# daultanigaurav/AI-BASED-FRAME-INTERPOLATION

Hardware: AMD Instinct MI355X
Metric: interpolated frames/sec at 1080p (higher is better)
Workload: dtype bf16

## Files before the change

### ai_based_frame_interpolation_amd/_native.py

```python
from __future__ import annotations

import ctypes
import os
import subprocess

import torch

_PKG = os.path.dirname(os.path.abspath(__file__))
LIB_PATH = os.environ.get("FIUNET_LIB") or os.path.join(_PKG, "libfiunet_hip.so")
CSRC = os.path.join(_PKG, "csrc")

ABI_VERSION = 8
ABI_MIN_COMPAT = 4
FP32, BF16, BF16X2, FP16 = 0, 1, 2, 3
OPT_UNFUSED, OPT_KEEP_ALL, OPT_GATHER_UPSAMPLE = 1, 2, 16
OPT_RNE_WEIGHTS, OPT_NO_DITHER = 32, 64
YUV_MPEG2, YUV_BT709, YUV_FULL_RANGE, YUV_BT2020 = 1, 2, 4, 8

SYMBOLS = (
    "fiunet_abi_version", "fiunet_last_error_string", "fiunet_create", "fiunet_destroy",
    "fiunet_set_options", "fiunet_load_weights", "fiunet_prepare_precision", "fiunet_workspace_bytes", "fiunet_forward",
    "fiunet_min_unsplit_batch",
    "fiunet_forward_strip",
    "fiunet_workspace_bytes_u8", "fiunet_forward_u8", "fiunet_forward_u8_strided", "fiunet_preprocess_u8",
    "fiunet_postprocess_u8", "fiunet_debug_read_activation", "fiunet_profile_enable",
    "fiunet_profile_read", "fiunet_metrics_workspace_bytes", "fiunet_psnr_u8", "fiunet_ssim_u8",
    "fiunet_ssim_gauss_workspace_bytes", "fiunet_ssim_gauss_f32",
    "fiunet_yuv420_to_rgb_u8", "fiunet_rgb_to_yuv420_u8", "fiunet_workspace_bytes_yuv420", "fiunet_forward_yuv420",
    "fiunet_preprocess_p10", "fiunet_postprocess_p10", "fiunet_workspace_bytes_p10", "fiunet_forward_p10",
    "fiunet_yuv420p10_to_rgb_p10", "fiunet_rgb_p10_to_yuv420p10", "fiunet_workspace_bytes_yuv420p10",
    "fiunet_forward_yuv420p10",
    "fiunet_pair_sad_u8", "fiunet_pair_sad_p10", "fiunet_scene_cuts", "fiunet_hold_cut_frames",
    "fiunet_retime_u8", "fiunet_retime_p10",
    "fiunet_nv12_to_rgb_u8", "fiunet_rgb_to_nv12_u8", "fiunet_workspace_bytes_nv12", "fiunet_forward_nv12",
    "fiunet_p010_to_rgb_p10", "fiunet_rgb_p10_to_p010", "fiunet_workspace_bytes_p010", "fiunet_forward_p010",
)


class SurfaceLayout(ctypes.Structure):
# ... 421 lines not shown
```

### ai_based_frame_interpolation_amd/csrc/conv3x3_mfma.hip.h

```cpp
#pragma once
#include <hip/hip_runtime.h>
#include <stdint.h>
#include <type_traits>

namespace fiunet {

typedef __attribute__((ext_vector_type(4))) float f32x4;
typedef __attribute__((ext_vector_type(8))) __bf16 bf16x8;
typedef __attribute__((ext_vector_type(8))) _Float16 f16x8;

enum SrcMode { SRC_DIRECT = 0, SRC_POOL = 1 , SRC_CONCAT_UP = 2,
               SRC_STEM = 3 ,
               SRC_DIRECT_X2 = 4,
               SRC_STEM_X2 = 5 };
constexpr bool src_is_stem(int mode) { return mode == SRC_STEM || mode == SRC_STEM_X2; }
constexpr bool src_is_x2(int mode) { return mode == SRC_DIRECT_X2 || mode == SRC_STEM_X2; }

__device__ __forceinline__ size_t blk_off(int plane, int y, int x, int H, int W)
{
    return (((size_t)plane * H + y) * W + x) * 64;
}

struct ConvArgs {
    const void* src0;
// ... 9 lines not shown
    int padT, padL;
    float sy, sx;
    int upOffY;
    int lowOffY;
    int lowHg;
    int tilesX, tilesY, nct;
    int relu;
    const float* f1;
    const float* f2;
    const void* stem_w;
    float dither;
    int ksplit;
    float* kslab;
    unsigned long long* stamp;
    unsigned stamp_cap;
    const float* head_w;
    const float* head_b;
    float* head_out;
    const uint8_t* u1;
    const uint8_t* u2;
    uint8_t* head_out_u8;
    int head_nc;
    size_t head_img_stride;
};

template <typename T> struct Elem;
template <> struct Elem<float> {
    static constexpr int PL = 16;
    static constexpr int NE = 4;
};
template <> struct Elem<__bf16> {
    static constexpr int PL = 32;
    static constexpr int NE = 8;
};
template <> struct Elem<_Float16> {
    static constexpr int PL = 32;
    static constexpr int NE = 8;
};

template <typename T> __device__ __forceinline__ void chunk_unpack(const uint4& c, float* f);
template <> __device__ __forceinline__ void chunk_unpack<float>(const uint4& c, float* f)
{
    f[0] = __uint_as_float(c.x); f[1] = __uint_as_float(c.y);
    f[2] = __uint_as_float(c.z); f[3] = __uint_as_float(c.w);
}
template <> __device__ __forceinline__ void chunk_unpack<__bf16>(const uint4& c, float* f)
// ... 320 lines not shown
    static constexpr int TAB_BYTES = MODE == SRC_CONCAT_UP ? ((THP + TW + 2) * 16 + 255) / 256 * 256 : 0;
    static constexpr int STEMW_OFF = TAB_OFF + TAB_BYTES;
    static constexpr int STEMW_BYTES = src_is_stem(MODE) ? 4096 : 0;
    static constexpr int LDS_BYTES = STEMW_OFF + STEMW_BYTES;
    static_assert(LDS_BYTES <= 80 * 1024, "two workgroups must fit in the CU's 160 KiB of LDS");
    static_assert(!src_is_stem(MODE) || LDS_BYTES <= 63 * 1280, "fused-stem kernel: stay below 64 LDS granules");
};

constexpr int conv_wave_frags(int BN, int TH, int TW) { return TH * TW / 16 / (4 / (BN / 64)); }
constexpr int conv_occupancy(int BN, int TH, int TW, int lds_bytes = 0)
{
    return conv_wave_frags(BN, TH, TW) == 4 && lds_bytes * 3 <= 160 * 1024 ? 3 : 2;
}


__device__ __forceinline__ int conv_block_remap()
{
    const int nblk = gridDim.x, bid = blockIdx.x;
    const int q = nblk >> 3, r = nblk & 7, xcd = bid & 7;
    return (xcd < r ? xcd * (q + 1) : r * (q + 1) + (xcd - r) * q) + (bid >> 3);
}

struct ConvTileId { int ct, b, ty, tx; };
__device__ __forceinline__ ConvTileId conv_tile_decode(const ConvArgs& a, int t)
{
    ConvTileId d;
    d.ct = t % a.nct; t /= a.nct;
    d.tx = t % a.tilesX; t /= a.tilesX;
    d.ty = t % a.tilesY;
    d.b = t / a.tilesY;
    return d;
}

template <typename T> __device__ __forceinline__ int conv_cout_ofs(int m, int lc)
{
    return sizeof(T) == 2 ? (m >> 1) * 32 + lc * 8 + (m & 1) * 4 : m * 16 + lc * 4;
}

template <typename T, int BN, int TH, int TW, int EPI>
__device__ __forceinline__ void conv_acc_init(const ConvArgs& a, f32x4 (&acc)[4][conv_wave_frags(BN, TH, TW)],
                                              int ct, int wc, int lc)
{
    constexpr int NF = conv_wave_frags(BN, TH, TW);
#pragma unroll
    for (int m = 0; m < 4; ++m) {
        f32x4 v = f32x4{0.f, 0.f, 0.f, 0.f};
        if constexpr (!epi_is_splitk(EPI)) {
            const float4 sh = *reinterpret_cast<const float4*>(a.shift + ct * BN + wc * 64 + conv_cout_ofs<T>(m, lc));
            v = f32x4{sh.x, sh.y, sh.z, sh.w};
        }
#pragma unroll
        for (int n = 0; n < NF; ++n) acc[m][n] = v;
    }
}
// ... 263 lines not shown
            } else {
#pragma unroll
                for (int g = 0; g < 2; ++g) {
                    unsigned r[4];
#pragma unroll
                    for (int h = 0; h < 2; ++h) {
                        const int m = 2 * g + h;
                        const unsigned a0 = pk_max_i16(pack2_pk<T>(acc[m][n][0], acc[m][n][1]),
                                                       pack2_pk<T>(acc[m][n + FR][0], acc[m][n + FR][1]));
                        const unsigned a1 = pk_max_i16(pack2_pk<T>(acc[m][n][2], acc[m][n][3]),
                                                       pack2_pk<T>(acc[m][n + FR][2], acc[m][n + FR][3]));
                        r[2 * h] = pk_max_i16(a0, dpp_swap_pairs(a0));
                        r[2 * h + 1] = pk_max_i16(a1, dpp_swap_pairs(a1));
                        if (a.relu) { r[2 * h] = relu_pk_bf16(r[2 * h]); r[2 * h + 1] = relu_pk_bf16(r[2 * h + 1]); }
                    }
                    if (okp) *reinterpret_cast<uint4*>(o + g * pplane_stride) = make_uint4(r[0], r[1], r[2], r[3]);
                }
            }
        }
    }
}

template <typename T, int BN, int TH, int TW, int MODE, int EPI>
__global__ __launch_bounds__(256, conv_occupancy(BN, TH, TW, ConvTile<BN, TH, TW, MODE>::LDS_BYTES)) void conv3x3_mfma_kernel(const ConvArgs a)
{
    using Tile = ConvTile<BN, TH, TW, MODE>;
    constexpr int PL = Elem<T>::PL;
    constexpr int TWP = Tile::TWP, THP = Tile::THP;
    constexpr int WAVES_C = BN / 64, WAVES_P = 4 / WAVES_C;
    constexpr int FR = TW / 16;
    constexpr int NF = conv_wave_frags(BN, TH, TW);
    constexpr int ROWS_W = NF / FR;
    static_assert(NF == 8 || NF == 4, "wave tile must be 64 couts x 128 or 64 pixels");
    static_assert(TH == ROWS_W * WAVES_P && ROWS_W * FR == NF, "tile does not split over the waves");
    static_assert(EPI != EPI_POOL || ROWS_W % 2 == 0, "pooled epilogue: a wave owns whole row pairs");
    static_assert(Tile::LDS_BYTES * conv_occupancy(BN, TH, TW, Tile::LDS_BYTES) <= 160 * 1024, "LDS per CU");
    constexpr int HNC = EPI == EPI_HEAD ? 1 : (EPI == EPI_HEAD3 ? 3 : 0);
    static_assert(HNC == 0 || BN == 64, "fused head needs all 64 couts in one wave");
    static_assert(MODE == SRC_DIRECT || MODE == SRC_CONCAT_UP || MODE == SRC_STEM || MODE == SRC_DIRECT_X2 ||
                  MODE == SRC_STEM_X2, "pooling is fused into the producer");
    constexpr bool X2 = src_is_x2(MODE);
    constexpr bool STEM = src_is_stem(MODE);
    constexpr bool DIRECT = MODE == SRC_DIRECT || MODE == SRC_DIRECT_X2;
    static_assert(!X2 || std::is_same_v<T, __bf16>, "two-piece operands are bf16");
    static_assert(!STEM || (sizeof(T) == 2 && BN == 64), "fused stem: 2-byte output (bf16 / fp16), 64 couts");

    extern __shared__ __attribute__((aligned(16))) char smem[];
    char* const lds_in = smem;
    char* const lds_w = smem + Tile::IN_BYTES;
    const unsigned lds_in_addr = lds_addr_of(lds_in);
    const unsigned lds_w_addr = lds_addr_of(lds_w);

    int lid = conv_block_remap();
    const int ksplit = epi_is_splitk(EPI) ? a.ksplit : 1;
    const int split = lid % ksplit;
    lid /= ksplit;
    const ConvTileId id = conv_tile_decode(a, lid);
    const int ct = id.ct, b = id.b;
    const int y0 = id.ty * TH, x0 = id.tx * TW;

    const int tid = threadIdx.x;
    const int lane = tid & 63, wave = __builtin_amdgcn_readfirstlane(tid >> 6);
    const int l15 = lane & 15, lc = lane >> 4;
    const int wc = wave % WAVES_C, wp = wave / WAVES_C;

#ifdef FIUNET_STAMP
    unsigned long long st_sum[16] = {0, 0, 0, 0, 0, 0, 0, 0, 0, 0, 0, 0, 0, 0, 0, 0};
    unsigned long long st_t0 = __builtin_amdgcn_s_memtime(), st_prev = st_t0;
#ifdef FIUNET_STAMP_PROLOG
    unsigned long long st_pprev = st_t0;
#define PSTAMP(slot) do { __builtin_amdgcn_sched_barrier(0); const unsigned long long t_ = __builtin_amdgcn_s_memtime(); \
                          st_sum[slot] += t_ - st_pprev; st_pprev = t_; __builtin_amdgcn_sched_barrier(0); } while (0)
#else
#define PSTAMP(slot) do {} while (0)
#endif
#define STAMP(slot) do { const unsigned long long t_ = __builtin_amdgcn_s_memtime(); \
                         st_sum[slot] += t_ - st_prev; st_prev = t_; } while (0)
#define STAMP_UP(slot) STAMP(slot)
#else
#define STAMP(slot) do {} while (0)
#define STAMP_UP(slot) do {} while (0)
#define PSTAMP(slot) do {} while (0)
// ... 525 lines not shown
        const unsigned long long ck_t1 = __builtin_amdgcn_s_memtime(), ck_r1 = __builtin_amdgcn_s_memrealtime();
        const unsigned st_idx = blockIdx.x * 4u + (unsigned)wave;
        if (a.stamp && lane == 0 && st_idx < a.stamp_cap) {
            unsigned long long* rec = a.stamp + (size_t)st_idx * 16;
            rec[0] = ck_t1 - ck_t0;
            rec[1] = ck_r1 - ck_r0;
            rec[8] = 1ull;
        }
    }
#endif
    conv_epilogue<T, BN, TH, TW, EPI, X2>(a, acc, b, y0, x0, ct, split, wc, wp, l15, lc);
#ifdef FIUNET_STAMP
    STAMP(5);
    st_sum[0] = st_prev - st_t0;
    const unsigned st_idx = blockIdx.x * 4u + (unsigned)wave;
    if (a.stamp && lane == 0 && st_idx < a.stamp_cap) {
        unsigned long long* rec = a.stamp + (size_t)st_idx * 16;
#pragma unroll
        for (int k = 0; k < 16; ++k) rec[k] = k == 8 ? 1ull : st_sum[k];
    }
#endif
}

template <typename T, int BN, int TH, int TW, int EPI, bool X2>
__global__ __launch_bounds__(64) void splitk_finalize_tile_kernel(const ConvArgs a)
{
    static_assert(EPI == EPI_PLAIN || EPI == EPI_POOL, "a fused head is never K-split");
    constexpr int WAVES_C = BN / 64;
    constexpr int NF = conv_wave_frags(BN, TH, TW);
    int t = blockIdx.x >> 2;
    const int tile = t;
    const int ct = t % a.nct; t /= a.nct;
    const int tx = t % a.tilesX; t /= a.tilesX;
    const int ty = t % a.tilesY;
    const int b = t / a.tilesY;
    const int lane = threadIdx.x & 63, wave = blockIdx.x & 3;
    const int l15 = lane & 15, lc = lane >> 4;
    const int wc = wave % WAVES_C, wp = wave / WAVES_C;
    const int ntile = a.B * a.tilesY * a.tilesX * a.nct;
    f32x4 acc[4][NF];
#pragma unroll
    for (int m = 0; m < 4; ++m)
#pragma unroll
        for (int n = 0; n < NF; ++n) acc[m][n] = f32x4{0.f, 0.f, 0.f, 0.f};
    const float4* p = reinterpret_cast<const float4*>(a.kslab) + (((size_t)tile * 4 + wave) * (4 * NF)) * 64 + lane;
    const size_t slice = (size_t)ntile * 4 * (4 * NF) * 64;
// ... 36 lines not shown
```

### ai_based_frame_interpolation_amd/csrc/fiunet.hip

```cpp
#include "../../include/fiunet.h"
#include "pointwise.hip.h"
#include "conv3x3_kwave.hip.h"
#include "metrics.hip.h"
#include "colour.hip.h"
#include "scene.hip.h"
#include "retime.hip.h"

#include <algorithm>
#include <atomic>
#include <cmath>
#include <cstdio>
#include <cstring>
#include <map>
#include <string>
#include <vector>

using namespace fiunet;

namespace {

thread_local std::string g_err;

int fail(int code, const std::string& msg)
{
// ... 146 lines not shown
    if (dev >= 0 && dev < 64 && !lds_attr_set[dev].load(std::memory_order_acquire)) {
        HIP_TRY(hipFuncSetAttribute(reinterpret_cast<const void*>(Kernel), hipFuncAttributeMaxDynamicSharedMemorySize, lds));
        lds_attr_set[dev].store(true, std::memory_order_release);
    }
    hipLaunchKernelGGL(Kernel, dim3((unsigned)nblk), dim3(256), lds, s, a);
    HIP_TRY(hipGetLastError());
    return FIUNET_OK;
}

template <typename T, int BN, int TH, int TW, int MODE, int EPI>
int launch_conv_cfg(ConvArgs a, hipStream_t s)
{
    char name[128] = "";
    if (g_name_out)
        std::snprintf(name, sizeof name, "conv3x3_mfma_kernel<%s,%d,%d,%d,%d,%d>", elem_name<T>(), BN, TH, TW,
                      MODE, EPI);
    a.tilesX = (a.W + TW - 1) / TW;
    a.tilesY = (a.H + TH - 1) / TH;
    a.nct = a.Cout / BN;
    const long long nblk = (long long)a.B * a.tilesX * a.tilesY * a.nct * (epi_is_splitk(EPI) ? a.ksplit : 1);
    return launch_lds<&conv3x3_mfma_kernel<T, BN, TH, TW, MODE, EPI>>(name, nblk, ConvTile<BN, TH, TW, MODE>::LDS_BYTES, a, s);
}

inline unsigned grid_for(size_t n) { return (unsigned)std::min<size_t>((n + 255) / 256, 256 * 32); }

inline long long padded_area(int H, int W, int TH, int TW)
{
    return (long long)((H + TH - 1) / TH) * TH * ((W + TW - 1) / TW) * TW;
}

inline bool prefer_wide(int H, int W, int THw, int TWw, int THn, int TWn)
{
    const long long wide = padded_area(H, W, THw, TWw), narrow = padded_area(H, W, THn, TWn);
    return wide * 32 <= narrow * 33;
}

struct TileShape { int BN, TH, TW; };
struct ConvCfg { bool small; int ksplit; bool kwave = false; };

inline TileShape big_tile(int H, int W, int Cout)
{
    if (Cout == 64) return prefer_wide(H, W, 16, 32, 32, 16) ? TileShape{64, 16, 32} : TileShape{64, 32, 16};
    return prefer_wide(H, W, 8, 32, 16, 16) ? TileShape{128, 8, 32} : TileShape{128, 16, 16};
}
constexpr TileShape kSmallTile = {64, 8, 32};

inline long long tile_blocks(const TileShape& t, int B, int H, int W, int Cout)
{
    return (long long)B * ((W + t.TW - 1) / t.TW) * ((H + t.TH - 1) / t.TH) * (Cout / t.BN);
}

inline int pow2_floor(long long v) { int k = 1; while (2LL * k <= v) k *= 2; return k; }

inline int small_ksplit(bool fp32, long long nblk, int nplanes, int fp32_slots = 256)
{
    int k;
    if (nblk >= (fp32 ? fp32_slots : 256)) return 1;
    if (fp32) k = pow2_floor(std::max<long long>(1, fp32_slots / std::max<long long>(nblk, 1)));
    else {
        k = nplanes < 8 ? 1 : (nplanes < 16 ? 4 : 8);
        k = std::min(k, pow2_floor(std::max<long long>(1, 512 / std::max<long long>(nblk, 1))));
    }
    k = std::min(k, pow2_floor(nplanes));
    while (k > 1 && (size_t)k * nblk * kSmallTile.BN * kSmallTile.TH * kSmallTile.TW * 4 > kSlabBytes) k /= 2;
    return k;
}

inline bool kwave_applies(int B, int H, int W, int Cin, int Cout)
{
    const TileShape big = big_tile(H, W, Cout);
    const long long nblk_big = tile_blocks(big, B, H, W, Cout);
    if (nblk_big >= 256 || !(nblk_big < (nblk_big / B < 64 ? 256 : 128))) return false;
    const long long nwg = (long long)B * ((H + 1) / 2) * ((W + 31) / 32) * (Cout / 64);
    return Cin / 32 >= 4 && Cout % 64 == 0 && nwg <= 256;
}

inline bool small_tile_wins_on_the_tail(long long nblk_big, long long nblk_small, double area_ratio)
{
    auto rounds = [](long long n, int slots, int occ) {
        const long long full = n / slots, rem = n % slots;
        return (double)full + (rem ? 0.2 + 0.8 * (double)((rem + 255) / 256) / occ : 0.0);
    };
    return rounds(nblk_small, 768, 3) * 0.81 * area_ratio < rounds(nblk_big, 512, 2);
}

inline ConvCfg choose_conv_cfg(bool fp32, bool x2, int B, int H, int W, int Cin, int Cout, bool splittable,
                               int force_small = -1, int force_ksplit = 0, bool kwave_ok = false, bool tail_rule_ok = false,
                               bool concat_conv = false)
{
    const int PL = fp32 ? 16 : 32;
    const int nplanes = Cin / PL * (x2 ? 3 : 1);
    const TileShape big = big_tile(H, W, Cout);
    const long long nblk_big = tile_blocks(big, B, H, W, Cout), nblk_small = tile_blocks(kSmallTile, B, H, W, Cout);
    if (nblk_big >= 256 && force_small < 0 && force_ksplit <= 0) {
        const bool small = tail_rule_ok && nblk_big <= 2304 &&
                           small_tile_wins_on_the_tail(nblk_big, nblk_small,
                                                       (double)padded_area(H, W, kSmallTile.TH, kSmallTile.TW) /
                                                           (double)padded_area(H, W, big.TH, big.TW));
        return ConvCfg{small, 1};
    }
    const bool may_split = splittable && nblk_big < (nblk_big / B < 64 ? 256 : 128);
    if (kwave_ok && fp32 && splittable && Cin / 16 >= 4 && force_small == 2) return ConvCfg{true, 1, true};
    if (kwave_ok && !fp32 && splittable && Cin / 32 >= 4 && (force_small == 2 || (force_small < 0 && force_ksplit <= 0))) {
        if (force_small == 2 || (kwave_applies(B, H, W, Cin, Cout) && !(x2 && Cin / 32 > 8))) return ConvCfg{true, 1, true};
    }
    if (force_small == 2) force_small = 1;
    auto big_ksplit = [&]() {
        int k = (int)std::min<long long>(std::min(nplanes / 2, 16), (256 + nblk_big - 1) / nblk_big);
        k = k > 1 ? pow2_floor(k) : 1;
        while (k > 1 && (size_t)k * nblk_big * big.BN * big.TH * big.TW * 4 > kSlabBytes) k /= 2;
        return k;
    };
    bool small = force_small >= 0 ? force_small != 0 : true;
    if (force_small < 0 && fp32) {
        const int slots = concat_conv ? 512 : 256;
        auto mfma_ns = [&](long long nblk, int k, double step_ns) {
            const long long nwg = nblk * k;
            return (double)((nwg + slots - 1) / slots) * ((nplanes + k - 1) / k * 3) * step_ns + (k > 1 ? 8000.0 : 0.0);
        };
        const int ks = may_split ? small_ksplit(true, nblk_small, nplanes, slots) : 1, kb = may_split ? big_ksplit() : 1;
        small = mfma_ns(nblk_small, ks, 2950.0) <= mfma_ns(nblk_big, kb, 5900.0);
        if (kwave_ok && splittable && may_split && nplanes >= 4 && Cout % 64 == 0) {
            const long long nwg = (long long)B * ((H + 1) / 2) * ((W + 31) / 32) * (Cout / 64);
            const double kw = (double)((nwg + 255) / 256) * ((nplanes + 3) / 4 * 3) * 2950.0;
            if (nwg <= 512 && kw < (small ? mfma_ns(nblk_small, ks, 2950.0) : mfma_ns(nblk_big, kb, 5900.0))) return ConvCfg{true, 1, true};
        }
    }
    const TileShape& t = small ? kSmallTile : big;
    const long long nblk = small ? nblk_small : nblk_big;
    int k = 1;
    if (force_ksplit > 0) {
        k = splittable ? std::min(pow2_floor(force_ksplit), pow2_floor(nplanes)) : 1;
        while (k > 1 && (size_t)k * nblk * t.BN * t.TH * t.TW * 4 > kSlabBytes) k /= 2;
    } else if (may_split) {
        k = small ? small_ksplit(fp32, nblk, nplanes, concat_conv ? 512 : 256) : big_ksplit();
    }
    return ConvCfg{small, k};
}

inline bool fp32_concat_takes_kwave(int B, int H, int W, int Cin, int Cout)
{
    return choose_conv_cfg(true, false, B, H, W, Cin, Cout, true, -1, 0, true, false, false).kwave;
}

enum StemForm {
    STEM_FUSED = 0,
    STEM_FIRST = 1,
    STEM_RGB_SPLIT = 2,
};
enum SrcForm {
    FORM_DIRECT = 0,
    FORM_POOL = 1,
    FORM_CONCAT_GATHER = 2,
    FORM_CONCAT_UP = 3,
    FORM_CONCAT_CONVT = 4,
    FORM_CONCAT_UPCAT = 5,
    FORM_STEM = 6,
};
struct StageLaunch {
    int form = FORM_DIRECT;
// ... 11 lines not shown
    bool stem_w = false;
    const int* force_tile = nullptr;
    const int* force_ksplit = nullptr;
};

inline int conv_cin(const int* cout, bool bilinear, int i)
{
    if (kMode[i] != SRC_CONCAT_UP) return cout[kSrc0[i]];
    return cout[kSrc0[i]] + (bilinear ? cout[kSrc1[i]] : cout[kSrc1[i]] / 2);
}

inline bool materialise_up(int precision, int B, int H, int W, int Cin, int Cout)
{
    if (precision == FIUNET_FP32) return fp32_concat_takes_kwave(B, H, W, Cin, Cout);
    if (Cout >= 256 && (long long)B * H * W >= 65536) return true;
    return kwave_applies(B, H, W, Cin, Cout);
}

void plan_stages(const NetDesc& n, int precision, int B, int H, int W, StageLaunch L[NCONV])
{
    const bool fp32 = precision == FIUNET_FP32, x2 = precision == FIUNET_BF16X2;
    const bool keep_all = n.flags & FIUNET_OPT_KEEP_ALL;
    const bool unfused = !x2 && (n.flags & FIUNET_OPT_UNFUSED), gather_up = !x2 && (n.flags & FIUNET_OPT_GATHER_UPSAMPLE);
    int hs[5] = {H}, ws[5] = {W};
    for (int k = 1; k < 5; ++k) { hs[k] = hs[k - 1] / 2; ws[k] = ws[k - 1] / 2; }
    const bool fuse_stem = !fp32 && n.cf == 1 && n.stem_w && !unfused && !(x2 && keep_all) && prefer_wide(H, W, 16, 32, 32, 16);
    L[0] = StageLaunch{};
    L[0].form = fuse_stem && !keep_all ? STEM_FUSED : n.cf == 3 && !fp32 ? STEM_RGB_SPLIT : STEM_FIRST;
    L[0].stored = L[0].form != STEM_FUSED;
    for (int i = 1; i < NCONV; ++i) {
        StageLaunch& st = L[i];
        st = StageLaunch{};
        const int h = hs[kLevel[i]], w = ws[kLevel[i]], cin = conv_cin(n.cout, n.bilinear, i), cout = n.cout[i];
        if (i == 1 && fuse_stem) st.form = FORM_STEM;
        else if (kMode[i] == SRC_POOL) st.form = FORM_POOL;
        else if (kMode[i] == SRC_CONCAT_UP) {
            if (!n.bilinear) st.form = FORM_CONCAT_CONVT;
            else if (x2) st.form = FORM_CONCAT_UP;
            else if (unfused) st.form = FORM_CONCAT_UPCAT;
            else st.form = !gather_up && materialise_up(precision, B, h, w, cin, cout) ? FORM_CONCAT_UP : FORM_CONCAT_GATHER;
        }
        if (kPoolOut[i] >= 0 && !unfused) st.epi = EPI_POOL;
        if (i == NCONV - 1 && !unfused) st.epi = n.cf == 1 ? EPI_HEAD : EPI_HEAD3;
        st.slab = i != NCONV - 1;
        st.stored = !(i == NCONV - 1 && st.epi != EPI_PLAIN && !keep_all);
        const bool stem = st.form == FORM_STEM, gather = st.form == FORM_CONCAT_GATHER, direct = !stem && !gather;
        const bool plain_or_pool = st.epi == EPI_PLAIN || st.epi == EPI_POOL;
        const bool as_gather = st.form == FORM_CONCAT_UPCAT && fp32 && !fp32_concat_takes_kwave(B, h, w, cin, cout);
        st.cfg = choose_conv_cfg(fp32, x2, B, h, w, cin, cout, !stem && plain_or_pool && st.slab,
                                 (n.force_tile ? n.force_tile[i] : 0) - 1, stem || !n.force_ksplit ? 0 : n.force_ksplit[i],
                                 direct && plain_or_pool && !as_gather, direct || (gather && cout >= 256), gather || as_gather);
    }
}

struct Plan {
    StageLaunch st[NCONV];
    int hs[5], ws[5];
    size_t act_off[NCONV];
    size_t pool_off[4];
    size_t scratch_off;
    size_t up_off[NCONV];
    size_t slab_off;
    size_t total;
};

bool make_plan(const NetDesc& n, int B, int H, int W, int precision, Plan& p)
{
    if (B < 1 || H < 16 || W < 16) return false;
    if ((long long)H * W >= (1LL << 26)) return false;
    plan_stages(n, precision, B, H, W, p.st);
    const bool keep_all = n.flags & FIUNET_OPT_KEEP_ALL;
    const size_t es = two_byte_elems(precision) ? 2 : 4;
    p.hs[0] = H; p.ws[0] = W;
    for (int k = 1; k < 5; ++k) { p.hs[k] = p.hs[k - 1] / 2; p.ws[k] = p.ws[k - 1] / 2; }
// ... 70 lines not shown
            k.ksplit = ksplit;
            int rc = launch_conv_cfg<T, BN, TH, TW, MODE, EPI_SPLITK>(k, s);
            if (rc) return rc;
            k.tilesX = (a.W + TW - 1) / TW;
            k.tilesY = (a.H + TH - 1) / TH;
            k.nct = a.Cout / BN;
            const long long ntile = (long long)a.B * k.tilesX * k.tilesY * k.nct;
            hipLaunchKernelGGL((splitk_finalize_tile_kernel<T, BN, TH, TW, EPI, src_is_x2(MODE)>), dim3((unsigned)(4 * ntile)), dim3(64), 0, s, k);
            HIP_TRY(hipGetLastError());
            if (g_name_out) *g_name_out += "+splitk" + std::to_string(ksplit);
            return FIUNET_OK;
        }
    }
    return launch_conv_cfg<T, BN, TH, TW, MODE, EPI>(a, s);
}

template <typename T, int MODE, int EPI> int launch_conv_shape(const ConvArgs& a, const ConvCfg& cfg, hipStream_t s)
{
    if (a.Cout != 64 && a.Cout % 128 != 0) return fail(FIUNET_ERR_INVALID_ARG, "Cout must be 64 or k*128");
    if ((EPI == EPI_HEAD || EPI == EPI_HEAD3) && a.Cout != 64) return fail(FIUNET_ERR_INVALID_ARG, "fused head needs Cout == 64");
    if constexpr ((MODE == SRC_DIRECT || MODE == SRC_DIRECT_X2) && (EPI == EPI_PLAIN || EPI == EPI_POOL)) {
        if (cfg.kwave) return launch_kwave<T, EPI, MODE == SRC_DIRECT_X2>(a, s);
    }
    if (cfg.small) return launch_conv_maybe_split<T, 64, 8, 32, MODE, EPI>(a, s, cfg.ksplit);
    if (a.Cout == 64) {
        const bool wide = prefer_wide(a.H, a.W, 16, 32, 32, 16);
        return wide ? launch_conv_maybe_split<T, 64, 16, 32, MODE, EPI>(a, s, cfg.ksplit)
                    : launch_conv_maybe_split<T, 64, 32, 16, MODE, EPI>(a, s, cfg.ksplit);
    }
    if constexpr (EPI != EPI_HEAD && EPI != EPI_HEAD3) {
        const bool wide = prefer_wide(a.H, a.W, 8, 32, 16, 16);
        return wide ? launch_conv_maybe_split<T, 128, 8, 32, MODE, EPI>(a, s, cfg.ksplit)
                    : launch_conv_maybe_split<T, 128, 16, 16, MODE, EPI>(a, s, cfg.ksplit);
    }
    return fail(FIUNET_ERR_INVALID_ARG, "fused head needs Cout == 64");
}

template <typename T> int launch_conv(const ConvArgs& a, int mode, int epi, const ConvCfg& cfg, hipStream_t s)
{
    constexpr int PL = Elem<T>::PL;
    if (a.C0 % PL || a.C1 % PL) return fail(FIUNET_ERR_INVALID_ARG, "channels not a plane multiple");
    if (mode == SRC_CONCAT_UP && epi == EPI_PLAIN) return launch_conv_shape<T, SRC_CONCAT_UP, EPI_PLAIN>(a, cfg, s);
    if (mode == SRC_DIRECT && epi == EPI_PLAIN) return launch_conv_shape<T, SRC_DIRECT, EPI_PLAIN>(a, cfg, s);
    if (mode == SRC_DIRECT && epi == EPI_HEAD) return launch_conv_shape<T, SRC_DIRECT, EPI_HEAD>(a, cfg, s);
    if (mode == SRC_DIRECT && epi == EPI_HEAD3) return launch_conv_shape<T, SRC_DIRECT, EPI_HEAD3>(a, cfg, s);
    if (mode == SRC_DIRECT && epi == EPI_POOL) return launch_conv_shape<T, SRC_DIRECT, EPI_POOL>(a, cfg, s);
// ... 1218 lines not shown
    return retime(grid, n_intervals, frame_samples, depth, first_interval, j0, n_out, p, q, mode, flags, out, stream);
}

int fiunet_retime_p10(const uint16_t* grid, int n_intervals, size_t frame_samples, int depth, uint64_t first_interval,
                      uint64_t j0, int n_out, uint32_t p, uint32_t q, int mode, const uint8_t* flags, uint16_t* out,
                      void* stream)
{
    return retime(grid, n_intervals, frame_samples, depth, first_interval, j0, n_out, p, q, mode, flags, out, stream);
}

int fiunet_debug_force_cfg(fiunet_ctx* ctx, int layer, int tile, int ksplit)
{
    if (!ctx || layer >= NCONV || tile < 0 || tile > 3 || ksplit < 0 || ksplit > 32)
        return fail(FIUNET_ERR_INVALID_ARG, "fiunet_debug_force_cfg: bad arguments");
    if (layer < 0) {
        for (int i = 0; i < NCONV; ++i) ctx->force_tile[i] = ctx->force_ksplit[i] = 0;
        return FIUNET_OK;
    }
    ctx->force_tile[layer] = tile;
    ctx->force_ksplit[layer] = ksplit;
    return FIUNET_OK;
}

int fiunet_debug_choose_cfg(int precision, int B, int H, int W, int Cin, int Cout, int splittable, int concat_stage,
                            int kwave_ok, int* out )
{
    if (!out || B < 1 || H < 1 || W < 1 || Cin < 32 || (Cout != 64 && Cout % 128 != 0) || !valid_precision(precision))
        return fail(FIUNET_ERR_INVALID_ARG, "fiunet_debug_choose_cfg: bad arguments");
    const bool concat = concat_stage >= 10;
    out[3] = concat && concat_stage < NCONV && kMode[concat_stage] == SRC_CONCAT_UP &&
             (precision == FIUNET_BF16X2 ||
              materialise_up(precision, B, H, W, conv_cin(kCoutBil, true, concat_stage), kCoutBil[concat_stage]));
    const ConvCfg c = choose_conv_cfg(precision == FIUNET_FP32, precision == FIUNET_BF16X2, B, H, W, Cin, Cout, splittable != 0,
                                      -1, 0, concat ? out[3] != 0 : kwave_ok != 0, kwave_ok != 0,
                                      concat && !(precision == FIUNET_FP32 && out[3]));
    out[0] = c.small; out[1] = c.ksplit; out[2] = c.kwave;
    return FIUNET_OK;
}

int fiunet_debug_stage_cfg(int frame_channels, int bilinear, unsigned flags, int precision, int B, int H, int W, int stage,
                           int* out )
{
    if (!out || (frame_channels != 1 && frame_channels != 3) || B < 1 || H < 16 || W < 16 || stage < 0 || stage >= NCONV ||
        !valid_precision(precision))
        return fail(FIUNET_ERR_INVALID_ARG, "fiunet_debug_stage_cfg: bad arguments");
    NetDesc n;
    n.cf = frame_channels;
    n.bilinear = bilinear != 0;
    n.cout = n.bilinear ? kCoutBil : kCoutCT;
    n.flags = flags;
    n.stem_w = frame_channels == 1;
    StageLaunch L[NCONV];
    plan_stages(n, precision, B, H, W, L);
    const StageLaunch& st = L[stage];
    out[0] = st.cfg.small; out[1] = st.cfg.ksplit; out[2] = st.cfg.kwave;
    out[3] = stage > 0 && (st.form == FORM_CONCAT_UP || st.form == FORM_CONCAT_CONVT);
    out[4] = st.form; out[5] = st.epi;
    return FIUNET_OK;
}

// ... 114 lines not shown
```

### ai_based_frame_interpolation_amd/unet.py

```python
from __future__ import annotations

import os

import torch
import torch.nn as nn

from . import _native

_ENCODER = (("down1", 64, 128), ("down2", 128, 256), ("down3", 256, 512), ("down4", 512, 512))
_DECODER = (("up1", 1024, 256), ("up2", 512, 128), ("up3", 256, 64), ("up4", 128, 64))
_ENCODER_CT = (("down1", 64, 128), ("down2", 128, 256), ("down3", 256, 512), ("down4", 512, 1024))
_DECODER_CT = (("up1", 1024, 512), ("up2", 512, 256), ("up3", 256, 128), ("up4", 128, 64))

TAP_CHANNELS = (64, 64, 128, 128, 256, 256, 512, 512, 512, 512, 512, 256, 256, 128, 128, 64, 64, 64)
TAP_CHANNELS_CT = (64, 64, 128, 128, 256, 256, 512, 512, 1024, 1024, 512, 512, 256, 256, 128, 128, 64, 64)
TAP_LEVEL = (0, 0, 1, 1, 2, 2, 3, 3, 4, 4, 3, 3, 2, 2, 1, 1, 0, 0)
TAP_NAMES = tuple(
    f"{p}.double_conv.{c}"
    for p in ("unet.inc", "unet.down1.maxpool_conv.1", "unet.down2.maxpool_conv.1",
              "unet.down3.maxpool_conv.1", "unet.down4.maxpool_conv.1", "unet.up1.conv",
              "unet.up2.conv", "unet.up3.conv", "unet.up4.conv")
    for c in (0, 3))

UP_TAP_NAMES = ("unet.up1.up", "unet.up2.up", "unet.up3.up", "unet.up4.up")

_PRECISIONS = {"fp32": _native.FP32, "float32": _native.FP32, "bf16x2": _native.BF16X2, "bf16": _native.BF16,
               "bfloat16": _native.BF16, "fp16": _native.FP16, "float16": _native.FP16, "half": _native.FP16}


class _Holder(nn.Module):

    def forward(self, *a, **k):
        raise RuntimeError("parameter holder: the forward runs in the HIP kernels, not in torch")


class _Slot(nn.Module):

    def __init__(self, what: str):
        super().__init__()
        self.what = what

    def extra_repr(self):
        return f"{self.what} (fused into the HIP conv kernels)"

    def forward(self, *a, **k):
        raise RuntimeError(f"{self.what}: fused into the HIP kernels, not callable on its own")


class _Seq(nn.ModuleDict):

# ... 49 lines not shown
            else:
                u.up = nn.ConvTranspose2d(cin, cin // 2, kernel_size=2, stride=2)
                u.conv = _double_conv(cin, cout)
            setattr(self, name, u)
        self.outc = _Holder()
        self.outc.conv = nn.Conv2d(64, n_classes, kernel_size=1)


class FrameInterpolationUNet(nn.Module):

    def __init__(self, bilinear: bool = False, frame_channels: int = 1, precision: str | None = None):
        super().__init__()
        self.unet = UNet(n_channels=2 * frame_channels, n_classes=frame_channels, bilinear=bilinear)
        self.frame_channels = frame_channels
        self.precision = precision or os.environ.get("FIUNET_PRECISION", "fp32")
        if self.precision not in _PRECISIONS:
            raise ValueError(f"precision must be one of {sorted(_PRECISIONS)}")
        self._ctx = None
        self._ctx_dirty = True
        self._weights_gen = 0
        self._tracked = None
        self._fingerprint = None
        self._ws = None
        self._options = 0

    def _apply(self, fn, *a, **k):
        self._ctx_dirty = True
        self._tracked = None
        return super()._apply(fn, *a, **k)

    def _current_fingerprint(self):
        tracked = list(self.parameters()) + list(self.buffers())
        fp = []
        for t in tracked:
            try:
                ver = t._version
            except RuntimeError:
                ver = 0
            fp.append((id(t), ver, t.data_ptr()))
        return tuple(fp)

    def __getstate__(self):
        st = self.__dict__.copy()
        st["_ctx"], st["_ws"], st["_tracked"], st["_fingerprint"], st["_ctx_dirty"] = None, None, None, None, True
        return st

    def __deepcopy__(self, memo):
        import copy
        new = self.__class__.__new__(self.__class__)
        memo[id(self)] = new
        for k, v in self.__getstate__().items():
            new.__dict__[k] = copy.deepcopy(v, memo)
        return new

    def load_state_dict(self, *a, **k):
        self._ctx_dirty = True
        self._tracked = None
        return super().load_state_dict(*a, **k)

    def refresh_weights(self):
        self._ctx_dirty = True

    def set_options(self, *, unfused: bool = False, keep_all: bool = False, gather_upsample: bool = False,
                    rne_weights: bool = False, no_dither: bool = False):
        old = self._options
        self._options = ((_native.OPT_UNFUSED if unfused else 0) | (_native.OPT_KEEP_ALL if keep_all else 0)
                         | (_native.OPT_GATHER_UPSAMPLE if gather_upsample else 0)
                         | (_native.OPT_RNE_WEIGHTS if rne_weights else 0)
                         | (_native.OPT_NO_DITHER if no_dither else 0))
        if (old ^ self._options) & _native.OPT_RNE_WEIGHTS:
            self._ctx_dirty = True
        if self._ctx is not None:
            self._ctx.set_options(self._options)

    def _ctx_or_none_set_options(self):
        if self._ctx is not None:
            self._ctx.set_options(self._options)

    def _context(self, device: torch.device) -> "_native.Context":
        idx = device.index if device.index is not None else torch.cuda.current_device()
        if self._ctx is None or self._ctx.device_index != idx:
            if self._ctx is not None:
                self._ctx.close()
            self._ctx = _native.Context(idx, self.frame_channels, self.unet.bilinear)
            self._ctx_dirty = True
        fp = self._current_fingerprint()
        if self._ctx_dirty or fp != self._fingerprint:
            self._ctx.set_options(self._options)
            self._ctx.load_state_dict(self.state_dict())
            self._ctx_dirty = False
            self._fingerprint = fp
            self._weights_gen += 1
# ... 285 lines not shown
```

### include/fiunet.h

```cpp
#ifndef FIUNET_H
#define FIUNET_H

#include <stddef.h>
#include <stdint.h>

#ifdef __cplusplus
extern "C" {
#endif

#define FIUNET_ABI_VERSION 8

enum fiunet_status {
    FIUNET_OK = 0,
    FIUNET_ERR_INVALID_ARG = 1,
    FIUNET_ERR_BAD_SHAPE = 2,
    FIUNET_ERR_MISSING_WEIGHT = 3,
    FIUNET_ERR_NOT_LOADED = 4,
    FIUNET_ERR_WORKSPACE = 5,
    FIUNET_ERR_HIP = 6,
    FIUNET_ERR_UNSUPPORTED = 7
};

enum fiunet_precision {
    FIUNET_FP32 = 0,
    FIUNET_BF16 = 1,
    FIUNET_BF16X2 = 2,
    FIUNET_FP16 = 3
};

enum fiunet_option {
    FIUNET_OPT_UNFUSED = 1,
    FIUNET_OPT_KEEP_ALL = 2,
    FIUNET_OPT_RNE_WEIGHTS = 32,
    FIUNET_OPT_NO_DITHER = 64,
    FIUNET_OPT_GATHER_UPSAMPLE = 16
};

typedef struct fiunet_ctx fiunet_ctx;

int fiunet_create(fiunet_ctx** out_ctx, int device_id, int frame_channels, int bilinear);

int fiunet_destroy(fiunet_ctx* ctx);

int fiunet_set_options(fiunet_ctx* ctx, unsigned flags);

int fiunet_load_weights(fiunet_ctx* ctx, int n, const char* const* names,
                        const float* const* host_ptrs, const int64_t* numels);

int fiunet_prepare_precision(fiunet_ctx* ctx, int precision);

size_t fiunet_workspace_bytes(const fiunet_ctx* ctx, int B, int H, int W, int precision);

int fiunet_min_unsplit_batch(const fiunet_ctx* ctx, int H, int W, int precision);

int fiunet_forward(fiunet_ctx* ctx, const float* frame1, const float* frame2, float* out, int B,
                   int H, int W, int precision, void* workspace, size_t workspace_bytes,
                   void* stream);

// ... 110 lines not shown
```

Measured before the change: 529.8.

## Launch mixed 8x32 main and 16x16 edge tiles in one conv grid

Adds a conv kernel that covers most of the image with 8x32 tiles and the leftover right column (when width mod 32 is 1..16) with 16x16 tiles, in a single launch. An XCD-aware remap splits workgroups between the main and edge regions. The aim is to avoid padded waste from partial 32-wide tiles on widths like 240, without falling back to small tiles everywhere. It adds an option flag and env var to disable it, plus a debug query for the chosen launch. It only applies to bf16/fp16 direct plain/pool convs, and most 1080p levels have widths divisible by 32.

```diff
diff --git a/ai_based_frame_interpolation_amd/_native.py b/ai_based_frame_interpolation_amd/_native.py
--- a/ai_based_frame_interpolation_amd/_native.py
+++ b/ai_based_frame_interpolation_amd/_native.py
@@ -14,7 +14,7 @@
 ABI_MIN_COMPAT = 4
 FP32, BF16, BF16X2, FP16 = 0, 1, 2, 3
 OPT_UNFUSED, OPT_KEEP_ALL, OPT_GATHER_UPSAMPLE = 1, 2, 16
-OPT_RNE_WEIGHTS, OPT_NO_DITHER = 32, 64
+OPT_RNE_WEIGHTS, OPT_NO_DITHER, OPT_NO_MIXED_TILES = 32, 64, 128
 YUV_MPEG2, YUV_BT709, YUV_FULL_RANGE, YUV_BT2020 = 1, 2, 4, 8
 
 SYMBOLS = (
diff --git a/ai_based_frame_interpolation_amd/csrc/conv3x3_mfma.hip.h b/ai_based_frame_interpolation_amd/csrc/conv3x3_mfma.hip.h
--- a/ai_based_frame_interpolation_amd/csrc/conv3x3_mfma.hip.h
+++ b/ai_based_frame_interpolation_amd/csrc/conv3x3_mfma.hip.h
@@ -55,6 +55,7 @@
     uint8_t* head_out_u8;
     int head_nc;
     size_t head_img_stride;
+    int nmain, etilesY, ex0;
 };
 
 template <typename T> struct Elem;
@@ -421,14 +422,36 @@
 }
 
 struct ConvTileId { int ct, b, ty, tx; };
+__device__ __forceinline__ ConvTileId conv_tile_decode(int nct, int tilesX, int tilesY, int t)
+{
+    ConvTileId d;
+    d.ct = t % nct; t /= nct;
+    d.tx = t % tilesX; t /= tilesX;
+    d.ty = t % tilesY;
+    d.b = t / tilesY;
+    return d;
+}
 __device__ __forceinline__ ConvTileId conv_tile_decode(const ConvArgs& a, int t)
 {
-    ConvTileId d;
-    d.ct = t % a.nct; t /= a.nct;
-    d.tx = t % a.tilesX; t /= a.tilesX;
-    d.ty = t % a.tilesY;
-    d.b = t / a.tilesY;
-    return d;
+    return conv_tile_decode(a.nct, a.tilesX, a.tilesY, t);
+}
+
+struct ConvRegionId { int lid; bool edge; };
+__device__ __forceinline__ ConvRegionId conv_mixed_remap(int nmain)
+{
+    const int nedge = (int)gridDim.x - nmain, bid = blockIdx.x;
+    const int xcd = bid & 7, k = bid >> 3;
+    const int qm = nmain >> 3, rm = nmain & 7, qe = nedge >> 3, re = nedge & 7;
+    const int cm = qm + (xcd < rm ? 1 : 0);
+    ConvRegionId r;
+    r.edge = k >= cm;
+    if (!r.edge) {
+        r.lid = xcd * qm + min(xcd, rm) + k;
+    } else {
+        const int e = (xcd - rm) & 7;
+        r.lid = e * qe + min(e, re) + (k - cm);
+    }
+    return r;
 }
 
 template <typename T> __device__ __forceinline__ int conv_cout_ofs(int m, int lc)
@@ -738,7 +761,7 @@
 }
 
 template <typename T, int BN, int TH, int TW, int MODE, int EPI>
-__global__ __launch_bounds__(256, conv_occupancy(BN, TH, TW, ConvTile<BN, TH, TW, MODE>::LDS_BYTES)) void conv3x3_mfma_kernel(const ConvArgs a)
+__device__ __forceinline__ void conv3x3_mfma_tile(const ConvArgs& a, int lid, int tilesX, int tilesY, int xorg)
 {
     using Tile = ConvTile<BN, TH, TW, MODE>;
     constexpr int PL = Elem<T>::PL;
@@ -767,13 +790,12 @@
     const unsigned lds_in_addr = lds_addr_of(lds_in);
     const unsigned lds_w_addr = lds_addr_of(lds_w);
 
-    int lid = conv_block_remap();
     const int ksplit = epi_is_splitk(EPI) ? a.ksplit : 1;
     const int split = lid % ksplit;
     lid /= ksplit;
-    const ConvTileId id = conv_tile_decode(a, lid);
+    const ConvTileId id = conv_tile_decode(a.nct, tilesX, tilesY, lid);
     const int ct = id.ct, b = id.b;
-    const int y0 = id.ty * TH, x0 = id.tx * TW;
+    const int y0 = id.ty * TH, x0 = xorg + id.tx * TW;
 
     const int tid = threadIdx.x;
     const int lane = tid & 63, wave = __builtin_amdgcn_readfirstlane(tid >> 6);
@@ -1345,6 +1367,27 @@
 #endif
 }
 
+template <typename T, int BN, int TH, int TW, int MODE, int EPI>
+__global__ __launch_bounds__(256, conv_occupancy(BN, TH, TW, ConvTile<BN, TH, TW, MODE>::LDS_BYTES)) void conv3x3_mfma_kernel(const ConvArgs a)
+{
+    conv3x3_mfma_tile<T, BN, TH, TW, MODE, EPI>(a, conv_block_remap(), a.tilesX, a.tilesY, 0);
+}
+
+template <typename T, int MODE, int EPI>
+__global__ __launch_bounds__(256, 2) void conv3x3_mixed_kernel(const ConvArgs a)
+{
+    static_assert(MODE == SRC_DIRECT && (EPI == EPI_PLAIN || EPI == EPI_POOL), "direct sources, plain or pooled epilogue");
+    static_assert(conv_occupancy(128, 8, 32) == 2 && conv_occupancy(128, 16, 16) == 2, "both bodies: two workgroups per CU");
+    const ConvRegionId r = conv_mixed_remap(a.nmain);
+    if (!r.edge) conv3x3_mfma_tile<T, 128, 8, 32, MODE, EPI>(a, r.lid, a.tilesX, a.tilesY, 0);
+    else conv3x3_mfma_tile<T, 128, 16, 16, MODE, EPI>(a, r.lid, 1, a.etilesY, a.ex0);
+}
+template <int MODE> constexpr int conv_mixed_lds_bytes()
+{
+    return ConvTile<128, 8, 32, MODE>::LDS_BYTES > ConvTile<128, 16, 16, MODE>::LDS_BYTES ? ConvTile<128, 8, 32, MODE>::LDS_BYTES
+                                                                                          : ConvTile<128, 16, 16, MODE>::LDS_BYTES;
+}
+
 template <typename T, int BN, int TH, int TW, int EPI, bool X2>
 __global__ __launch_bounds__(64) void splitk_finalize_tile_kernel(const ConvArgs a)
 {
diff --git a/ai_based_frame_interpolation_amd/csrc/fiunet.hip b/ai_based_frame_interpolation_amd/csrc/fiunet.hip
--- a/ai_based_frame_interpolation_amd/csrc/fiunet.hip
+++ b/ai_based_frame_interpolation_amd/csrc/fiunet.hip
@@ -192,6 +192,22 @@
     return launch_lds<&conv3x3_mfma_kernel<T, BN, TH, TW, MODE, EPI>>(name, nblk, ConvTile<BN, TH, TW, MODE>::LDS_BYTES, a, s);
 }
 
+template <typename T, int MODE, int EPI>
+int launch_conv_mixed(ConvArgs a, int mainX, int etilesY, long long nmain, long long nedge, hipStream_t s)
+{
+    char name[128] = "";
+    if (g_name_out)
+        std::snprintf(name, sizeof name, "conv3x3_mixed_kernel<%s,128,8x32,16x16,%d,%d>", elem_name<T>(), MODE, EPI);
+    if (nmain + nedge > 0x7fffffffLL) return fail(FIUNET_ERR_INVALID_ARG, "conv grid too large");
+    a.tilesX = mainX;
+    a.tilesY = (a.H + 7) / 8;
+    a.nct = a.Cout / 128;
+    a.nmain = (int)nmain;
+    a.etilesY = etilesY;
+    a.ex0 = 32 * mainX;
+    return launch_lds<&conv3x3_mixed_kernel<T, MODE, EPI>>(name, nmain + nedge, conv_mixed_lds_bytes<MODE>(), a, s);
+}
+
 inline unsigned grid_for(size_t n) { return (unsigned)std::min<size_t>((n + 255) / 256, 256 * 32); }
 
 inline long long padded_area(int H, int W, int TH, int TW)
@@ -206,7 +222,8 @@
 }
 
 struct TileShape { int BN, TH, TW; };
-struct ConvCfg { bool small; int ksplit; bool kwave = false; };
+struct ConvCfg { bool small; int ksplit; bool kwave = false;
+                 bool mixed = false; };
 
 inline TileShape big_tile(int H, int W, int Cout)
 {
@@ -218,6 +235,20 @@
 inline long long tile_blocks(const TileShape& t, int B, int H, int W, int Cout)
 {
     return (long long)B * ((W + t.TW - 1) / t.TW) * ((H + t.TH - 1) / t.TH) * (Cout / t.BN);
+}
+
+inline bool mixed_tiles_fit(bool fp32, bool x2, int H, int W, int Cout)
+{
+    return !fp32 && !x2 && Cout % 128 == 0 && W > 32 && W % 32 >= 1 && W % 32 <= 16 && prefer_wide(H, W, 8, 32, 16, 16);
+}
+struct MixedGrid { int mainX, tilesY, etilesY, ex0; long long nmain, nedge; };
+inline MixedGrid mixed_grid(int B, int H, int W, int Cout)
+{
+    MixedGrid g;
+    g.mainX = W / 32; g.tilesY = (H + 7) / 8; g.etilesY = (H + 15) / 16; g.ex0 = 32 * g.mainX;
+    g.nmain = (long long)B * g.tilesY * g.mainX * (Cout / 128);
+    g.nedge = (long long)B * g.etilesY * (Cout / 128);
+    return g;
 }
 
 inline int pow2_floor(long long v) { int k = 1; while (2LL * k <= v) k *= 2; return k; }
@@ -256,8 +287,9 @@
 
 inline ConvCfg choose_conv_cfg(bool fp32, bool x2, int B, int H, int W, int Cin, int Cout, bool splittable,
                                int force_small = -1, int force_ksplit = 0, bool kwave_ok = false, bool tail_rule_ok = false,
-                               bool concat_conv = false)
-{
+                               bool concat_conv = false, bool mixed_ok = false)
+{
+    const bool mixed = mixed_ok && mixed_tiles_fit(fp32, x2, H, W, Cout);
     const int PL = fp32 ? 16 : 32;
     const int nplanes = Cin / PL * (x2 ? 3 : 1);
     const TileShape big = big_tile(H, W, Cout);
@@ -267,6 +299,7 @@
                            small_tile_wins_on_the_tail(nblk_big, nblk_small,
                                                        (double)padded_area(H, W, kSmallTile.TH, kSmallTile.TW) /
                                                            (double)padded_area(H, W, big.TH, big.TW));
+        if (mixed && !(small && B == 1 && nblk_big > 512)) return ConvCfg{false, 1, false, true};
         return ConvCfg{small, 1};
     }
     const bool may_split = splittable && nblk_big < (nblk_big / B < 64 ? 256 : 128);
@@ -305,7 +338,7 @@
     } else if (may_split) {
         k = small ? small_ksplit(fp32, nblk, nplanes, concat_conv ? 512 : 256) : big_ksplit();
     }
-    return ConvCfg{small, k};
+    return ConvCfg{small, k, false, mixed && !small && k == 1};
 }
 
 inline bool fp32_concat_takes_kwave(int B, int H, int W, int Cin, int Cout)
@@ -363,6 +396,7 @@
     const bool fp32 = precision == FIUNET_FP32, x2 = precision == FIUNET_BF16X2;
     const bool keep_all = n.flags & FIUNET_OPT_KEEP_ALL;
     const bool unfused = !x2 && (n.flags & FIUNET_OPT_UNFUSED), gather_up = !x2 && (n.flags & FIUNET_OPT_GATHER_UPSAMPLE);
+    const bool mixed_on = !(n.flags & FIUNET_OPT_NO_MIXED_TILES);
     int hs[5] = {H}, ws[5] = {W};
     for (int k = 1; k < 5; ++k) { hs[k] = hs[k - 1] / 2; ws[k] = ws[k - 1] / 2; }
     const bool fuse_stem = !fp32 && n.cf == 1 && n.stem_w && !unfused && !(x2 && keep_all) && prefer_wide(H, W, 16, 32, 32, 16);
@@ -390,7 +424,8 @@
         const bool as_gather = st.form == FORM_CONCAT_UPCAT && fp32 && !fp32_concat_takes_kwave(B, h, w, cin, cout);
         st.cfg = choose_conv_cfg(fp32, x2, B, h, w, cin, cout, !stem && plain_or_pool && st.slab,
                                  (n.force_tile ? n.force_tile[i] : 0) - 1, stem || !n.force_ksplit ? 0 : n.force_ksplit[i],
-                                 direct && plain_or_pool && !as_gather, direct || (gather && cout >= 256), gather || as_gather);
+                                 direct && plain_or_pool && !as_gather, direct || (gather && cout >= 256), gather || as_gather,
+                                 mixed_on && direct && plain_or_pool);
     }
 }
 
@@ -507,6 +542,13 @@
     if constexpr ((MODE == SRC_DIRECT || MODE == SRC_DIRECT_X2) && (EPI == EPI_PLAIN || EPI == EPI_POOL)) {
         if (cfg.kwave) return launch_kwave<T, EPI, MODE == SRC_DIRECT_X2>(a, s);
     }
+    if constexpr (MODE == SRC_DIRECT && (EPI == EPI_PLAIN || EPI == EPI_POOL) && sizeof(T) == 2) {
+        if (cfg.mixed) {
+            const MixedGrid g = mixed_grid(a.B, a.H, a.W, a.Cout);
+            return launch_conv_mixed<T, MODE, EPI>(a, g.mainX, g.etilesY, g.nmain, g.nedge, s);
+        }
+    }
+    if (cfg.mixed) return fail(FIUNET_ERR_INVALID_ARG, "internal: mixed-tile launch planned for a form it does not cover");
     if (cfg.small) return launch_conv_maybe_split<T, 64, 8, 32, MODE, EPI>(a, s, cfg.ksplit);
     if (a.Cout == 64) {
         const bool wide = prefer_wide(a.H, a.W, 16, 32, 32, 16);
@@ -1771,20 +1813,44 @@
     return FIUNET_OK;
 }
 
-int fiunet_debug_choose_cfg(int precision, int B, int H, int W, int Cin, int Cout, int splittable, int concat_stage,
-                            int kwave_ok, int* out )
-{
-    if (!out || B < 1 || H < 1 || W < 1 || Cin < 32 || (Cout != 64 && Cout % 128 != 0) || !valid_precision(precision))
-        return fail(FIUNET_ERR_INVALID_ARG, "fiunet_debug_choose_cfg: bad arguments");
+static int debug_choose(int precision, int B, int H, int W, int Cin, int Cout, int splittable, int concat_stage, int kwave_ok,
+                        unsigned flags, int out[6])
+{
     const bool concat = concat_stage >= 10;
     out[3] = concat && concat_stage < NCONV && kMode[concat_stage] == SRC_CONCAT_UP &&
              (precision == FIUNET_BF16X2 ||
               materialise_up(precision, B, H, W, conv_cin(kCoutBil, true, concat_stage), kCoutBil[concat_stage]));
-    const ConvCfg c = choose_conv_cfg(precision == FIUNET_FP32, precision == FIUNET_BF16X2, B, H, W, Cin, Cout, splittable != 0,
+    const bool fp32 = precision == FIUNET_FP32, x2 = precision == FIUNET_BF16X2;
+    const bool mixed_ok = !(flags & FIUNET_OPT_NO_MIXED_TILES) && splittable != 0 && (!concat || out[3] != 0);
+    const ConvCfg c = choose_conv_cfg(fp32, x2, B, H, W, Cin, Cout, splittable != 0,
                                       -1, 0, concat ? out[3] != 0 : kwave_ok != 0, kwave_ok != 0,
-                                      concat && !(precision == FIUNET_FP32 && out[3]));
-    out[0] = c.small; out[1] = c.ksplit; out[2] = c.kwave;
-    return FIUNET_OK;
+                                      concat && !(precision == FIUNET_FP32 && out[3]), mixed_ok);
+    out[0] = c.small; out[1] = c.ksplit; out[2] = c.kwave; out[4] = c.mixed;
+    long long nwg;
+    if (c.mixed) { const MixedGrid g = mixed_grid(B, H, W, Cout); nwg = g.nmain + g.nedge; }
+    else if (c.kwave) nwg = (long long)B * ((H + KWaveTile::TH - 1) / KWaveTile::TH) * ((W + KWaveTile::TW - 1) / KWaveTile::TW) * (Cout / KWaveTile::BN);
+    else nwg = tile_blocks(c.small ? kSmallTile : big_tile(H, W, Cout), B, H, W, Cout) * c.ksplit;
+    out[5] = nwg > 0x7fffffffLL ? 0 : (int)nwg;
+    return FIUNET_OK;
+}
+
+int fiunet_debug_choose_cfg(int precision, int B, int H, int W, int Cin, int Cout, int splittable, int concat_stage,
+                            int kwave_ok, int* out )
+{
+    if (!out || B < 1 || H < 1 || W < 1 || Cin < 32 || (Cout != 64 && Cout % 128 != 0) || !valid_precision(precision))
+        return fail(FIUNET_ERR_INVALID_ARG, "fiunet_debug_choose_cfg: bad arguments");
+    int o[6];
+    debug_choose(precision, B, H, W, Cin, Cout, splittable, concat_stage, kwave_ok, 0u, o);
+    for (int k = 0; k < 4; ++k) out[k] = o[k];
+    return FIUNET_OK;
+}
+
+int fiunet_debug_choose_launch(int precision, int B, int H, int W, int Cin, int Cout, int splittable, int concat_stage,
+                               int kwave_ok, unsigned flags, int* out )
+{
+    if (!out || B < 1 || H < 1 || W < 1 || Cin < 32 || (Cout != 64 && Cout % 128 != 0) || !valid_precision(precision))
+        return fail(FIUNET_ERR_INVALID_ARG, "fiunet_debug_choose_launch: bad arguments");
+    return debug_choose(precision, B, H, W, Cin, Cout, splittable, concat_stage, kwave_ok, flags, out);
 }
 
 int fiunet_debug_stage_cfg(int frame_channels, int bilinear, unsigned flags, int precision, int B, int H, int W, int stage,
diff --git a/ai_based_frame_interpolation_amd/unet.py b/ai_based_frame_interpolation_amd/unet.py
--- a/ai_based_frame_interpolation_amd/unet.py
+++ b/ai_based_frame_interpolation_amd/unet.py
@@ -26,6 +26,10 @@
 
 _PRECISIONS = {"fp32": _native.FP32, "float32": _native.FP32, "bf16x2": _native.BF16X2, "bf16": _native.BF16,
                "bfloat16": _native.BF16, "fp16": _native.FP16, "float16": _native.FP16, "half": _native.FP16}
+
+
+def _env_options() -> int:
+    return _native.OPT_NO_MIXED_TILES if os.environ.get("FIUNET_NO_MIXED_TILES") == "1" else 0
 
 
 class _Holder(nn.Module):
@@ -121,7 +125,7 @@
         self._tracked = None
         self._fingerprint = None
         self._ws = None
-        self._options = 0
+        self._options = _env_options()
 
     def _apply(self, fn, *a, **k):
         self._ctx_dirty = True
@@ -161,12 +165,14 @@
         self._ctx_dirty = True
 
     def set_options(self, *, unfused: bool = False, keep_all: bool = False, gather_upsample: bool = False,
-                    rne_weights: bool = False, no_dither: bool = False):
+                    rne_weights: bool = False, no_dither: bool = False, no_mixed_tiles: "bool | None" = None):
         old = self._options
         self._options = ((_native.OPT_UNFUSED if unfused else 0) | (_native.OPT_KEEP_ALL if keep_all else 0)
                          | (_native.OPT_GATHER_UPSAMPLE if gather_upsample else 0)
                          | (_native.OPT_RNE_WEIGHTS if rne_weights else 0)
-                         | (_native.OPT_NO_DITHER if no_dither else 0))
+                         | (_native.OPT_NO_DITHER if no_dither else 0)
+                         | (_env_options() if no_mixed_tiles is None else
+                            _native.OPT_NO_MIXED_TILES if no_mixed_tiles else 0))
         if (old ^ self._options) & _native.OPT_RNE_WEIGHTS:
             self._ctx_dirty = True
         if self._ctx is not None:
diff --git a/include/fiunet.h b/include/fiunet.h
--- a/include/fiunet.h
+++ b/include/fiunet.h
@@ -33,7 +33,8 @@
     FIUNET_OPT_KEEP_ALL = 2,
     FIUNET_OPT_RNE_WEIGHTS = 32,
     FIUNET_OPT_NO_DITHER = 64,
-    FIUNET_OPT_GATHER_UPSAMPLE = 16
+    FIUNET_OPT_GATHER_UPSAMPLE = 16,
+    FIUNET_OPT_NO_MIXED_TILES = 128
 };
 
 typedef struct fiunet_ctx fiunet_ctx;
```

After: 536.2, median of 6. Within noise of the previous version (+1.2%).
